# lmjakt/kmer_hasheR

Measured on AMD Instinct MI355X. Metric: Mbp/s indexed (make.kmer.hash k=31) at 1/2/4/8 GPUs; seq.kmer.pos query Mbp/s, higher is better.
Workload: dtype u64; 1 GPU; configs[1]: synthetic 10 Mbp iid ACGT (splitmix64 seed 1+rank), k=31, make.kmer.hash index build; self seq.kmer.pos query timed alongside; seq_len=10000000, k=31, distinct_kmers=9999970, positions=9999970, parallelism=single

## Files before the change

### kmer_hasher_amd/csrc/kmhg_engine.cpp

```cpp
#include <atomic>
#include <hip/hip_runtime.h>
#include <sys/mman.h>

#include <algorithm>
#include <climits>
#include <cmath>
#include <cstdio>
#include <cstdlib>
#include <cstring>
#include <exception>
#include <functional>
#include <map>
#include <memory>
#include <mutex>
#include <numeric>
#include <string>
#include <thread>
#include <vector>

#include "kmhg_common.h"
#include "kmhg_blocks.h"
#include "kmhg_chains.h"
#include "kmhg_kernels.h"
#include "kmhg_plan.h"
#include "kmhg_hostwork.h"
#include "kmhg_pool.h"
#include "kmhg_reads.h"
#include "kmhg_querycall.h"
#include "kmhg_segrec.h"
#include "kmhg_parts_read.h"
#include "kmhg_fastx.h"
#include "kmhg_khash.h"
#include "kmhg_sh.h"

namespace kmhg {
inline const char* test_build_knob(const char* name) {
#ifdef KMHG_TEST_BUILD
  return std::getenv(name);
#else
  (void)name;
  return nullptr;
#endif
}
}
#include "../../include/kmhgpu.h"

using namespace kmhg;

static thread_local std::string g_err;

namespace {

struct Error {
  int code;
  std::string msg;
};

[[noreturn]] void fail(int code, const std::string& msg) { throw Error{code, msg}; }

void hip_check(hipError_t e, const char* what) {
  if (e != hipSuccess) {
    if (e == hipErrorOutOfMemory) fail(KMHG_ENOMEM, std::string(what) + ": out of device memory");
    fail(KMHG_EDEVICE, std::string(what) + ": " + hipGetErrorString(e));
  }
}
#define HIPC(x) hip_check((x), #x)

template <class F>
int guarded(F&& f) {
  try {
    f();
    return KMHG_OK;
  } catch (const Error& e) {
    g_err = e.msg;
    return e.code;
  } catch (const std::bad_alloc&) {
    g_err = "host allocation failed";
    return KMHG_ENOMEM;
  }
}

struct HipDev {
  static PoolKnobs knobs() {
    PoolKnobs kn;
    if (const char* e = test_build_knob("KMHG_POOL_DEPTH"))
      kn.depth = (size_t)std::max(1, std::min(8, std::atoi(e)));
    if (const char* e = test_build_knob("KMHG_POOL_BESTFIT")) kn.best_fit = e[0] != '0';
    kn.trace = test_build_knob("KMHG_POOL_TRACE") != nullptr;
    return kn;
  }
  int current() { int dev = 0; HIPC(hipGetDevice(&dev)); return dev; }
  void use(int dev) { (void)hipSetDevice(dev); }
  PoolAlloc alloc(size_t sz, void** p, std::string* text) {
    const hipError_t e = hipMalloc(p, sz);
    if (e == hipSuccess) return PoolAlloc::ok;
    if (e == hipErrorOutOfMemory) { (void)hipGetLastError(); return PoolAlloc::oom; }
    *text = hipGetErrorString(e);
    return PoolAlloc::error;
  }
  void free(void* p) { (void)hipFree(p); }
  void* event() {
    hipEvent_t ev = nullptr;
    if (hipEventCreateWithFlags(&ev, hipEventDisableTiming | hipEventDisableSystemFence) ==
        hipSuccess)
      return ev;
    (void)hipGetLastError();
    return hipEventCreateWithFlags(&ev, hipEventDisableTiming) == hipSuccess ? ev : nullptr;
  }
  bool record(void* ev, void* s) {
    return hipEventRecord(static_cast<hipEvent_t>(ev), static_cast<hipStream_t>(s)) == hipSuccess;
  }
  bool done(void* ev) { return hipEventQuery(static_cast<hipEvent_t>(ev)) == hipSuccess; }
  void wait_event(void* ev) { (void)hipEventSynchronize(static_cast<hipEvent_t>(ev)); }
  void wait_stream(void* s) { (void)hipStreamSynchronize(static_cast<hipStream_t>(s)); }
  [[noreturn]] void alloc_failed(PoolAlloc st, const std::string& text) {
    if (st == PoolAlloc::oom) fail(KMHG_ENOMEM, "hipMalloc: out of device memory");
    fail(KMHG_EDEVICE, "hipMalloc: " + text);
  }
};
using DevicePool = BlockPool<HipDev>;
using ReleaseGroup = ReleaseGroupT<HipDev>;

template <class T>
struct DBuf {
  T* p = nullptr;
  size_t n = 0;
  hipStream_t s = nullptr;
  bool ordered = false;
  DBuf() = default;
  explicit DBuf(size_t count) { reset(count); }
  DBuf(size_t count, hipStream_t stream) { reset(count); bind(stream); }
  ~DBuf() { free(); }
  DBuf(const DBuf&) = delete;
  DBuf& operator=(const DBuf&) = delete;
  void bind(hipStream_t stream) { s = stream; ordered = true; }
  void reset(size_t count) {
    free();
    n = count;
    p = static_cast<T*>(DevicePool::get().alloc(std::max<size_t>(count, 1) * sizeof(T)));
  }
  void free() {
    if (p) DevicePool::get().release(p, s, ordered);
    p = nullptr; n = 0;
  }
  size_t bytes() const { return n * sizeof(T); }
  void swap_with(DBuf& o) {
    std::swap(p, o.p);
    std::swap(n, o.n);
    std::swap(s, o.s);
    std::swap(ordered, o.ordered);
  }
};

struct PinnedRec {
  BuildMeta* meta = nullptr;
  hipEvent_t ev = nullptr;
};
class PinnedPool {
 public:
  static PinnedPool& get() {
    static PinnedPool p;
    return p;
  }
  PinnedRec take() {
    std::lock_guard<std::mutex> g(mu_);
    for (size_t i = 0; i < pending_.size();) {
      if (hipEventQuery(pending_[i].ev) == hipSuccess) {
        free_.push_back(pending_[i]);
        pending_[i] = pending_.back();
        pending_.pop_back();
      } else {
        ++i;
      }
    }
    if (free_.empty()) {
      constexpr int kSlots = 64;
      BuildMeta* blk = nullptr;
      HIPC(hipHostMalloc(reinterpret_cast<void**>(&blk), sizeof(BuildMeta) * kSlots,
                         hipHostMallocCoherent));
      for (int i = 0; i < kSlots; ++i) {
        PinnedRec r;
        r.meta = blk + i;
        HIPC(hipEventCreateWithFlags(&r.ev, hipEventDisableTiming));
        free_.push_back(r);
      }
    }
    PinnedRec r = free_.back();
    free_.pop_back();
    std::memset(r.meta, 0, sizeof(*r.meta));
    return r;
  }
  void give(PinnedRec r, bool in_flight) {
    if (!r.meta) return;
    std::lock_guard<std::mutex> g(mu_);
    (in_flight ? pending_ : free_).push_back(r);
  }

 private:
  std::mutex mu_;
  std::vector<PinnedRec> free_, pending_;
};
struct GiveBack {
  PinnedRec& r;
  hipStream_t s;
  ~GiveBack() {
    if (std::uncaught_exceptions() > 0) (void)hipStreamSynchronize(s);
    PinnedPool::get().give(r, false);
  }
};

struct Timing {
  static Timing& get() {
    static Timing t;
    return t;
  }
  bool on = false;
  std::string only;
  struct Rec { std::string name; hipEvent_t a, b; };
  std::vector<Rec> recs;
  std::map<std::string, std::pair<int64_t, double>> acc;
  std::mutex mu;

  Timing() {
    const char* e = std::getenv("KMHG_TIMING");
    on = e && e[0] == '1';
  }
  std::vector<hipEvent_t> pool;
  hipEvent_t take() {
    if (!pool.empty()) { hipEvent_t e = pool.back(); pool.pop_back(); return e; }
    hipEvent_t e;
    if (hipEventCreateWithFlags(&e, hipEventDisableSystemFence) != hipSuccess) {
      (void)hipGetLastError();
      HIPC(hipEventCreate(&e));
    }
    return e;
  }
  template <class F>
  void run(const char* name, hipStream_t s, F&& launch) {
    if (!on || (!only.empty() && only != name)) { launch(); HIPC(hipGetLastError()); return; }
    hipEvent_t a, b;
    {
      std::lock_guard<std::mutex> g(mu);
      a = take();
      b = take();
    }
    HIPC(hipEventRecord(a, s));
    launch();
    HIPC(hipGetLastError());
    HIPC(hipEventRecord(b, s));
    std::lock_guard<std::mutex> g(mu);
    recs.push_back({name, a, b});
  }
  void collect() {
    std::lock_guard<std::mutex> g(mu);
    for (auto& r : recs) {
      (void)hipEventSynchronize(r.b);
      float ms = 0.f;
      (void)hipEventElapsedTime(&ms, r.a, r.b);
      auto& x = acc[r.name];
      x.first += 1;
      x.second += ms;
      pool.push_back(r.a);
      pool.push_back(r.b);
    }
    recs.clear();
  }
};
#define LAUNCH(name, stream, ...) Timing::get().run(name, stream, [&] { __VA_ARGS__; })

hipStream_t lib_stream() {
  static std::mutex mu;
  static std::map<int, hipStream_t> streams;
  int dev = 0;
  HIPC(hipGetDevice(&dev));
  std::lock_guard<std::mutex> g(mu);
  auto it = streams.find(dev);
  if (it != streams.end()) return it->second;
  hipStream_t s;
  HIPC(hipStreamCreateWithFlags(&s, hipStreamNonBlocking));
  streams[dev] = s;
  return s;
}

static bool fresh_threads() {
  const char* pe = test_build_knob("KMHG_HOST_POOL");
  return pe && pe[0] == '0';
}

constexpr size_t D2H_CHUNK = 16u << 20;
constexpr size_t D2H_STAGE_MIN = 4u << 20;
static int d2h_threads() {
  static const int n = [] {
    const char* e = std::getenv("KMHG_D2H_THREADS");
    return e ? std::max(1, std::min(16, std::atoi(e))) : 8;
  }();
  return n;
}

static void host_copy_par(char* dst, const char* src, size_t n) {
  for_stripes(n, d2h_threads(), 4096, fresh_threads(),
              [=](uint64_t a, uint64_t b) { std::memcpy(dst + a, src + a, b - a); });
}

struct PinStage {
  std::mutex mu;
  char* pin[2] = {nullptr, nullptr};
};
static PinStage& pin_stage() {
  static std::mutex map_mu;
  static std::map<int, PinStage> stages;
  int dev = 0;
  HIPC(hipGetDevice(&dev));
  std::lock_guard<std::mutex> g(map_mu);
  return stages[dev];
}

static void hint_huge_pages(void* dst, size_t bytes) {
  static const bool on = [] {
    const char* e = test_build_knob("KMHG_D2H_HUGE");
    return !(e && e[0] == '0');
  }();
  const Span h = on ? huge_span(dst, bytes) : Span{0, 0};
  if (h.len) (void)madvise(reinterpret_cast<void*>(h.begin), h.len, MADV_HUGEPAGE);
}

void d2h_host(void* dst, const void* src, size_t bytes, hipStream_t s) {
  if (!bytes) return;
  static const bool staged = [] {
    const char* e = test_build_knob("KMHG_D2H");
    return !(e && std::string(e) == "direct");
  }();
  hint_huge_pages(dst, bytes);
  if (!staged || bytes < D2H_STAGE_MIN) {
    HIPC(hipMemcpyAsync(dst, src, bytes, hipMemcpyDeviceToHost, s));
    HIPC(hipStreamSynchronize(s));
    return;
  }
  PinStage& st = pin_stage();
  std::lock_guard<std::mutex> g(st.mu);
  char** pin = st.pin;
  if (!pin[0])
    for (int i = 0; i < 2; ++i)
      HIPC(hipHostMalloc(reinterpret_cast<void**>(&pin[i]), D2H_CHUNK, hipHostMallocPortable));
  struct Ev2 {
    hipEvent_t e[2] = {nullptr, nullptr};
    hipStream_t s;
    ~Ev2() {
      if (std::uncaught_exceptions() > 0) (void)hipStreamSynchronize(s);
      for (auto x : e)
        if (x) (void)hipEventDestroy(x);
    }
  } evs{{nullptr, nullptr}, s};
  hipEvent_t* ev = evs.e;
// ... 217 lines not shown
    }
  });
  const size_t n = effective_len(seq, L);
  copy.join();
  if (err.code != KMHG_OK) fail(err.code, err.msg);
  return n;
}

void check_build_args(size_t L, int k) {
  if (k < 1 || k > 32) fail(KMHG_EINVAL, "k must be a positive integer less than 1+MAX_K");
  if ((int64_t)L <= k) fail(KMHG_EINVAL, "the length of the sequence must be at least k");
  if (L >= (size_t)INT32_MAX) fail(KMHG_EOVERFLOW, "sequence longer than 2^31-1 (int positions)");
}

QueryCall checked(const QueryCall& c) {
  if (c.code != KMHG_OK) fail(c.code, c.text);
  return c;
}

void check_query_args(size_t L, int k) { checked(query_call(L, k)); }

template <class F>
Error for_parts(const std::vector<int>& key, F&& fn) {
  const int n = (int)key.size();
  std::vector<Error> errs(n, Error{KMHG_OK, ""});
  std::vector<int> uniq;
  for (int d : key)
    if (std::find(uniq.begin(), uniq.end(), d) == uniq.end()) uniq.push_back(d);
  auto run_key = [&](int d) {
    for (int i = 0; i < n; ++i) {
      if (key[i] != d) continue;
      try {
        fn(i);
      } catch (const Error& e) {
        errs[i] = e;
      } catch (const std::bad_alloc&) {
        errs[i] = Error{KMHG_ENOMEM, "host allocation failed"};
      }
    }
  };
  std::vector<std::thread> th;
  for (size_t u = 1; u < uniq.size(); ++u) th.emplace_back(run_key, uniq[u]);
  if (!uniq.empty()) run_key(uniq[0]);
  for (auto& t : th) t.join();
  for (const Error& e : errs)
    if (e.code != KMHG_OK) return e;
  return Error{KMHG_OK, ""};
}

kmhg_index* build_device_v1(const uint8_t* d_seq, int64_t L, int k, hipStream_t s) {
  ReleaseGroup rg(s);
  auto idx = std::make_unique<kmhg_index>();
  idx->stream = s;
  idx->build_kind = KMHG_BUILD_GLOBAL;
  HIPC(hipGetDevice(&idx->device));
  idx->k = k;
  idx->L = L;
  const int64_t Nw = L - k + 1;
  const bool aligned = (reinterpret_cast<uintptr_t>(d_seq) & 15) == 0;
  idx->geom = Geom{1u, (uint32_t)table_capacity(Nw)};
  const uint64_t nslots = idx->slots();
  idx->table.reset(nslots);
  DBuf<uint32_t> win_slot(Nw, s);
  LAUNCH("k_table_init", s, launch_table_init(idx->table.p, nslots, s));
  LAUNCH("k_build_insert", s,
         launch_build_insert(d_seq, L, k, idx->table.p, idx->geom, win_slot.p, Nw, aligned, s));
  const uint32_t nt = tiles_for(nslots);
  const size_t scratch_bytes = (size_t)nt * 8 + 64 + sizeof(BuildMeta);
  DBuf<uint8_t> scratch(scratch_bytes, s);
  HIPC(hipMemsetAsync(scratch.p, 0, scratch_bytes, s));
  uint64_t* status = reinterpret_cast<uint64_t*>(scratch.p);
  uint32_t* ticket = reinterpret_cast<uint32_t*>(scratch.p + (size_t)nt * 8);
  BuildMeta* meta = reinterpret_cast<BuildMeta*>(scratch.p + (size_t)nt * 8 + 64);
  DBuf<uint64_t> ukeys(Nw, s);
  DBuf<uint32_t> counts(Nw, s), offsets(Nw + 1, s);
  DBuf<uint32_t> small_ids(Nw / 2 + 1, s), large_ids(Nw / LARGE_MIN + 1, s);
  LAUNCH("k_build_compact", s,
         launch_build_compact(idx->table.p, nslots, status, ticket, ukeys.p, counts.p,
                              offsets.p, small_ids.p, large_ids.p, meta, s));
  idx->positions.reset(Nw);
  LAUNCH("k_build_scatter", s, launch_build_scatter(win_slot.p, Nw, idx->table.p,
                                                    idx->positions.p, s));
  LAUNCH("k_sort_small", s, launch_sort_small(small_ids.p, meta, counts.p, offsets.p,
                                              idx->positions.p, s));
  LAUNCH("k_sort_large", s,
         launch_sort_large(large_ids.p, meta, counts.p, offsets.p, idx->positions.p,
                           reinterpret_cast<int32_t*>(win_slot.p), s));
  LAUNCH("k_inline_singles", s, launch_inline_singles(idx->table.p, nslots, idx->positions.p, s));
  BuildMeta hm;
  HIPC(hipMemcpyAsync(&hm, meta, sizeof(hm), hipMemcpyDeviceToHost, s));
  HIPC(hipStreamSynchronize(s));
  idx->U = hm.n_kmers;
  idx->N = hm.n_positions;
  idx->P = hm.n_pairs;
  idx->max_n = hm.max_count;
  return idx.release();
}

BuildKnobs read_build_knobs() {
  BuildKnobs kn;
  for (const char* name : BUILD_KNOB_NAMES)
    if (const char* v = test_build_knob(name)) set_build_knob(kn, name, v);
  return kn;
}

uint32_t bucket_round_of_current_device() {
  static std::atomic<uint32_t> cache[64];
  int dev = 0;
  if (hipGetDevice(&dev) != hipSuccess || dev < 0) return 0;
  if (dev < 64) {
    if (uint32_t v = cache[dev].load(std::memory_order_relaxed)) return v;
  }
  int cus = 0;
  if (hipDeviceGetAttribute(&cus, hipDeviceAttributeMultiprocessorCount, dev) != hipSuccess)
    cus = 0;
  const uint32_t v = (uint32_t)std::max(cus, 0) * (uint32_t)KMHG_BUCKET_WGS;
  if (dev < 64) cache[dev].store(v, std::memory_order_relaxed);
  return v;
}

#ifdef KMHG_TEST_BUILD
static std::mutex g_place_mu;
static uint32_t* g_place_ctr = nullptr;
static int g_place_dev = -1;
uint32_t* bucket_place_counters() {
  std::lock_guard<std::mutex> lk(g_place_mu);
  int dev = 0;
  HIPC(hipGetDevice(&dev));
  if (!g_place_ctr) {
    HIPC(hipMalloc(&g_place_ctr, 3 * sizeof(uint32_t)));
    HIPC(hipMemset(g_place_ctr, 0, 3 * sizeof(uint32_t)));
    g_place_dev = dev;
  }
  return dev == g_place_dev ? g_place_ctr : nullptr;
}
#else
uint32_t* bucket_place_counters() { return nullptr; }
#endif

#ifdef KMHG_TEST_BUILD
static std::atomic<uint64_t> g_bid_pack_ctr[2];
void count_bid_pack(bool packed) { g_bid_pack_ctr[packed ? 0 : 1].fetch_add(1, std::memory_order_relaxed); }
#else
void count_bid_pack(bool) {}
#endif

struct StreamPtrs {
  const uint8_t* d_seq = nullptr;
  const uint64_t* d_keys = nullptr;
};

kmhg_index* build_device_v2(const BuildRequest& rq, const StreamPtrs& in, hipStream_t s) {
  ReleaseGroup rg(s);
  const BuildKnobs kn = read_build_knobs();
  const BuildPlan P = plan_build(rq, kn, bucket_round_of_current_device());
  if (P.err != KMHG_OK) fail(P.err, P.msg);
  auto idx = std::make_unique<kmhg_index>();
  idx->stream = s;
  HIPC(hipGetDevice(&idx->device));
  idx->build_kind = ballot_ranks() ? KMHG_BUILD_PARTITIONED_BALLOT : KMHG_BUILD_PARTITIONED;
  idx->k = rq.k;
  idx->L = rq.L;
  idx->is_part = P.is_part;
  idx->geom = P.geom;
  if (P.empty_part) {
    idx->table.reset(1);
    idx->positions.reset(1);
    return idx.release();
  }
  const int k = rq.k;
  const int64_t L = rq.L, Nw = P.Nw;
  const bool from_keys = P.from_keys, co_auto = P.co_auto, bid = P.bid, partc = P.partc;
  const uint32_t passes = P.passes, R = P.R, ntiles = P.ntiles, nb = P.geom.nb;
  const uint64_t nhist = P.nhist;
  const Geom g = P.geom;
  auto mk_digit = [&](uint32_t dv, uint32_t r) { return make_digit(dv, r, P.digit32 ? g.nb : 0u); };
  const uint64_t* d_keys = in.d_keys;
  const uint8_t* d_seq = in.d_seq;
  DBuf<uint8_t> aligned_copy;
  if (!from_keys && (reinterpret_cast<uintptr_t>(d_seq) & 15) != 0) {
    aligned_copy.reset((size_t)L);
    aligned_copy.bind(s);
    HIPC(hipMemcpyAsync(aligned_copy.p, d_seq, (size_t)L, hipMemcpyDeviceToDevice, s));
    d_seq = aligned_copy.p;
  }
  if (bid) count_bid_pack(P.bid_pack);
  auto kwords = [&](int sd) { return ((uint64_t)(Nw + PTILE) * P.key_bytes[sd] + 7) / 8; };
  DBuf<uint64_t> kA(kwords(0), s), kB(kwords(1), s);
  DBuf<uint32_t> pA(P.pos_array[0] ? Nw + PTILE : 1, s), pB(P.pos_array[1] ? Nw + PTILE : 1, s);
  auto kptr = [&](int p) -> void* {
    return p < 0 && from_keys ? const_cast<uint64_t*>(d_keys) : P.side(p) ? kB.p : kA.p;
  };
  auto pptr = [&](int p) { return P.side(p) ? pB.p : pA.p; };
  const uint32_t pad = (uint32_t)Nw;
  DBuf<uint32_t> hist(nhist, s);
  DBuf<uint32_t> start((uint64_t)nb + 1, s);
  DBuf<uint32_t> segb(P.pack8 ? (uint64_t)R * (P.nseg8 + 1) : 1, s);
  DBuf<uint16_t> dsb(P.ds_on ? ((uint64_t)Nw + PTILE + 8) / (P.ds8 ? 2 : 1) + 8 : 1, s);
  uint8_t* ds8p = P.ds8 ? reinterpret_cast<uint8_t*>(dsb.p) : nullptr;
  uint16_t* ds16p = P.ds8 ? nullptr : dsb.p;
  const Pack8 pk8{P.pack8 ? P.sh8 : 0, segb.p, P.nseg8, mk_digit(1, R)};
  const size_t off_meta = 64, off_status = 128;
  const uint32_t n_status = P.scan_tiles + 1;
  const size_t scratch_bytes = off_status + (size_t)n_status * 8;
  DBuf<uint8_t> scratch(scratch_bytes, s);
  uint8_t* sc = scratch.p;
  uint32_t* n_valid = reinterpret_cast<uint32_t*>(sc);
  BuildMeta* meta = reinterpret_cast<BuildMeta*>(sc + off_meta);
  uint64_t* status = reinterpret_cast<uint64_t*>(sc + off_status);
  idx->rec = PinnedPool::get().take();
  if (!co_auto) idx->table.reset(idx->slots());
  idx->positions.reset(P.no_pos ? 1 : Nw);
  idx->bstats.reset(nb);
  DBuf<uint32_t> hll_rows(co_auto ? (size_t)ntiles * (HLL_REGS / 4) : 1, s);
  DBuf<uint32_t> hll_regs(co_auto ? HLL_PART_WORDS : 1, s);
  PinnedRec hrec;
  if (co_auto) hrec = PinnedPool::get().take();

  DBuf<uint32_t> lo_save(passes >= 2 ? R : 1, s);
  uint64_t r_top = 1;
  for (uint32_t i = 1; i < passes; ++i) r_top *= R;
  DBuf<uint32_t> lvA(passes >= 3 ? r_top + 1 : 1, s), lvB(passes >= 4 ? r_top + 1 : 1, s);
  uint32_t div = 1;
  DiagBlock db{nullptr, nullptr, nullptr};
  DBuf<uint32_t> tcnt(partc ? ntiles : 1, s);
  if (from_keys) {
    HIPC(hipMemsetD32Async(reinterpret_cast<hipDeviceptr_t>(n_valid), (int)Nw, 1, s));
    HIPC(hipMemsetAsync(meta, 0, sizeof(BuildMeta), s));
  } else {
    if (rq.codes) {
      idx->dcodes.reset(diag_block_words(Nw));
      db = idx->diag_block_of();
    }
    LAUNCH("k_v2_hist0", s,
           launch_v2_hist0(d_seq, L, k, Nw, g, mk_digit(1, R), hist.p, ntiles, status,
                           n_status, meta, s, db.code, db.nbit,
                           bid ? static_cast<uint32_t*>(kptr(-1)) : nullptr,
                           partc ? kB.p : nullptr, partc ? pB.p : nullptr,
                           partc ? tcnt.p : nullptr));
    if (partc) {
      LAUNCH("k_scan_u32", s, launch_scan_u32(tcnt.p, ntiles, status, n_valid, s));
    } else {
      LAUNCH("k_scan_u32", s, launch_scan_u32(hist.p, nhist, status, n_valid, s));
      const DigitOut ds0{ds16p, mk_digit(R, R), ds8p};
      LAUNCH("k_v2_scatter_seq", s,
             launch_v2_scatter(bid ? ScatterIn::first_pass(kptr(-1), Nw)
                                   : ScatterIn::sequence(d_seq, L, k, Nw),
                               P.F(-1), P.F(0), kptr(0), pptr(0), pad, n_valid, g, mk_digit(1, R),
                               hist.p, ntiles, s, nullptr, P.pack8 ? &pk8 : nullptr,
                               P.ds_out(0) ? &ds0 : nullptr));
      if (P.pack8)
        LAUNCH("k_seg_bounds", s,
               launch_seg_bounds(hist.p, ntiles, R, P.nseg8, (uint32_t)(P.seg8 / PTILE), n_valid,
                                 segb.p, s));
      div = R;
    }
  }
  uint32_t* hp = hist.p;
  uint32_t C = ntiles, nst = n_status;
  uint64_t nh = nhist;
  DBuf<uint32_t> hist1;
  if (rq.n_parts >= 2 && (passes > 1 || partc)) {
    uint32_t nv = 0;
    HIPC(hipMemcpyAsync(&nv, n_valid, 4, hipMemcpyDeviceToHost, s));
    HIPC(hipStreamSynchronize(s));
    C = std::max<uint32_t>(1u, (uint32_t)(((uint64_t)nv + PTILE - 1) / PTILE));
    nh = (uint64_t)R * C;
    nst = tiles_for(nh) + 1;
    hist1.reset(nh);
    hist1.bind(s);
    hp = hist1.p;
    if (!partc)
      HIPC(hipMemcpy2DAsync(lo_save.p, 4, hist.p, (size_t)ntiles * 4, 4, R,
                            hipMemcpyDeviceToDevice, s));
  }
  if (partc)
    LAUNCH("k_part_dense", s, launch_part_dense(kB.p, pB.p, tcnt.p, ntiles, n_valid, kptr(-1),
                                                pptr(-1), P.F(-1), s));
  uint32_t* save1 = hp == hist.p || partc ? lo_save.p : nullptr;
  auto level_of = [&](uint32_t p, uint32_t spread) {
    uint64_t dv = 1;
    for (uint32_t i = 0; i < p; ++i) dv *= R;
    const bool last = p + 1 == passes;
    const uint32_t* lin = p == 1 ? lo_save.p : ((p - 1) % 2 ? lvA.p : lvB.p);
    uint32_t* lout = last ? start.p : (p % 2 ? lvA.p : lvB.p);
    return BoundsFuse{lin, lout, mk_digit((uint32_t)dv, R), (uint32_t)dv, spread,
                      last ? g.nb : (uint32_t)(dv * R)};
  };
  auto launch_level = [&](uint32_t p, const BoundsFuse& f) {
    LAUNCH("k_v2_bounds", s,
           launch_v2_bounds_lo(P.F((int)p - 1), kptr((int)p - 1), n_valid, g, f.Dlast, f.div, hp, C,
                               f.lo_start, f.spread, f.start, f.nlim, s, pk8.sh));
  };
  for (uint32_t p = P.first_pass; p < passes; ++p) {
    const Digit Dp = mk_digit(div, R);
    const bool keys0 = from_keys && p == 0;
    const bool last = p + 1 == passes;
    const bool hll = co_auto && p == 0;
    const int pi = (int)p - 1;
    if (keys0)
      LAUNCH("k_v2_hist", s,
             launch_v2_hist_keys0(d_keys, n_valid, g, Dp, hp, C, status, nst, s,
                                  hll ? hll_rows.p : nullptr, hll ? hll_regs.p : nullptr,
                                  rq.skip_empty));
    else
      LAUNCH("k_v2_hist", s,
             launch_v2_hist(!P.ds_out(pi) ? P.F(pi)
                            : P.ds8       ? StreamFmt::Digits8
                                          : StreamFmt::Digits16,
                            P.ds_out(pi) ? dsb.p : kptr(pi), n_valid, g, Dp, hp, C, status, nst, s,
                            p == 1 ? save1 : nullptr, pk8.sh));
    LAUNCH("k_scan_u32", s, launch_scan_u32(hp, nh, status, n_valid, s));
    if (hll) {
      LAUNCH("k_v2_hll", s, launch_v2_hll(hll_rows.p, ntiles, hll_regs.p,
                                          &hrec.meta->distinct_est, n_valid,
                                          &hrec.meta->n_positions, s));
      HIPC(hipEventRecord(hrec.ev, s));
    }
    const BoundsFuse lv = level_of(p, 1u);
    const DigitOut dsn{ds16p, mk_digit(div * R, R), ds8p};
    LAUNCH("k_v2_scatter", s,
           launch_v2_scatter(keys0 ? ScatterIn::first_pass(d_keys, Nw, rq.skip_empty)
                                   : ScatterIn::stream(kptr(pi), pptr(pi)),
                             P.F(pi), P.F((int)p), kptr((int)p), pptr((int)p), pad, n_valid, g, Dp,
                             hp, C, s, P.fused(p) ? &lv : nullptr, P.pack8 ? &pk8 : nullptr,
                             P.ds_out((int)p) ? &dsn : nullptr));
    if (p >= 1 && !P.fused(p) && !last) launch_level(p, lv);
    div *= R;
  }
  const int last_p = (int)passes - 1;
  Geom gb = g;
  if (co_auto) {
    HIPC(hipEventSynchronize(hrec.ev));
    idx->co_est = hrec.meta->distinct_est;
    const uint64_t n_keys_valid = hrec.meta->n_positions;
    PinnedPool::get().give(hrec, false);
    idx->co_spread = co_spread_for(idx->co_est, n_keys_valid, kn.co_spread);
    gb = Geom{nb / (uint32_t)idx->co_spread, V2_CAPW};
    idx->geom = gb;
    idx->table.reset(idx->slots());
  }
  if (passes == 1) {
    LAUNCH("k_v2_bounds", s,
           launch_v2_bounds_lo(StreamFmt::Keys, nullptr, n_valid, g, mk_digit(1, R), 1u,
                               partc ? hp : hist.p, partc ? C : ntiles, nullptr, g.nb / gb.nb,
                               start.p, g.nb, s));
  } else if (!P.fused(passes - 1)) {
    launch_level(passes - 1, level_of(passes - 1, g.nb / gb.nb));
  }
#ifdef KMHG_STAMPS
  static uint64_t* stamps = nullptr;
  if (!stamps) HIPC(hipMallocManaged(&stamps, sizeof(uint64_t) * 8 * (1u << 22)));
  HIPC(hipMemsetAsync(stamps, 0, sizeof(uint64_t) * 8 * nb, s));
  kmhg::set_stamp_buffer(stamps);
#endif
  if (kn.test_disorder && !P.no_pos)
    launch_v2_test_disorder(P.F(last_p), kptr(last_p), pptr(last_p), start.p, n_valid,
                            kn.test_disorder, s);
  uint8_t* tg = nullptr;
  uint32_t* rep = nullptr;
  if (P.want_tags) {
    try {
      idx->ptag.reset(idx->slots() + 32);
      idx->ptag.bind(s);
      tg = idx->ptag.p;
      rep = db.uniq;
      HIPC(hipMemsetAsync(rep, 0, diag_uniq_words(Nw) * 4, s));
      HIPC(hipMemsetAsync(tg + idx->slots() - 1, 0, 33, s));
    } catch (const Error& e) {
      if (e.code != KMHG_ENOMEM) throw;
      (void)hipGetLastError();
      tg = nullptr;
      rep = nullptr;
    }
  }
  LAUNCH("k_v2_bucket_wg", s,
         launch_v2_bucket_wg(P.F(last_p), kptr(last_p), pptr(last_p), start.p, gb, idx->table.p,
                             idx->positions.p, idx->bstats.p, meta, s, n_valid, (uint32_t)Nw,
                             db.code, k, tg, rep, kn.bucket_place, bucket_place_counters()));
  idx->tags_built = tg != nullptr;
  LAUNCH("k_v2_stats", s, launch_v2_stats(idx->bstats.p, gb.nb, n_valid, meta, idx->rec.meta, s));
  idx->bstats_nb = gb.nb;
  HIPC(hipEventRecord(idx->rec.ev, s));
  rg.adopt(idx->rec.ev);
#ifdef KMHG_STAMPS
  if (const char* f = std::getenv("KMHG_STAMP_FILE")) {
    HIPC(hipStreamSynchronize(s));
    if (FILE* fp = fopen(f, "wb")) { fwrite(stamps, 8, 8 * (size_t)nb, fp); fclose(fp); }
  }
#endif
  idx->pending = true;
  idx->src = in.d_seq;
  return idx.release();
}

bool tags_on() {
  const char* e = test_build_knob("KMHG_QUERY_TAGS");
  return !(e && e[0] == '0');
}

static std::atomic<int> g_lane_state[64];
static std::mutex g_lane_mu;
static void lane_order_run(int blocks, uint64_t* bad, uint64_t* checked) {
  struct Probe {
    hipStream_t st = nullptr;
    unsigned long long* res = nullptr;
  };
  static Probe probes[64];
  int dev = 0;
  HIPC(hipGetDevice(&dev));
  Probe& pr = probes[(unsigned)dev % 64];
  if (!pr.st) HIPC(hipStreamCreateWithFlags(&pr.st, hipStreamNonBlocking));
  if (!pr.res) HIPC(hipMalloc(&pr.res, 2 * sizeof(unsigned long long)));
  unsigned long long h[2] = {0, 0};
  hipError_t e = hipMemsetAsync(pr.res, 0, sizeof(h), pr.st);
  if (e == hipSuccess) {
    launch_lane_order_check(pr.res, pr.st, blocks);
    e = hipMemcpyAsync(h, pr.res, sizeof(h), hipMemcpyDeviceToHost, pr.st);
  }
  if (e == hipSuccess) e = hipStreamSynchronize(pr.st);
  hip_check(e, "LDS lane-order check");
  *bad = h[0];
  *checked = h[1];
}
bool lane_ballot() {
  if (const char* e = test_build_knob("KMHG_TEST_BALLOT"))
    if (e[0] == '1') return true;
  int dev = 0;
  HIPC(hipGetDevice(&dev));
  std::atomic<int>& st = g_lane_state[(unsigned)dev % 64];
  int v = st.load(std::memory_order_acquire);
  if (v == 0) {
    std::lock_guard<std::mutex> lk(g_lane_mu);
    v = st.load(std::memory_order_relaxed);
    if (v == 0) {
      uint64_t bad = 0, chk = 0;
      lane_order_run(256, &bad, &chk);
      v = (bad == 0 && chk > 0) ? 1 : 2;
      st.store(v, std::memory_order_release);
    }
  }
  return v == 2;
}

int build_version() {
  const char* e = test_build_knob("KMHG_BUILD");
  return (e && std::string(e) == "v1") ? 1 : 2;
}

kmhg_index* build_device(const uint8_t* d_seq, int64_t L, int k, hipStream_t s, bool codes = true) {
  if (const char* e = test_build_knob("KMHG_DIAG_CODES"))
    if (e[0] == '0') codes = false;
  if (build_version() == 2)
    return build_device_v2(BuildRequest::sequence(L, k, codes), StreamPtrs{d_seq, nullptr}, s);
  return build_device_v1(d_seq, L, k, s);
}

void finish_build(kmhg_index* idx) {
  if (!idx->pending) return;
  HIPC(hipEventSynchronize(idx->rec.ev));
  const BuildMeta hm = *idx->rec.meta;
  PinnedPool::get().give(idx->rec, false);
  idx->rec = PinnedRec{};
  idx->pending = false;
  const uint8_t* src = idx->src;
  idx->src = nullptr;
  if (hm.overflow) {
    if (idx->is_part) fail(KMHG_EOVERFLOW, "a bucket of a part build overflowed its LDS table");
    std::unique_ptr<kmhg_index> v1(build_device_v1(src, idx->L, idx->k, idx->stream));
    idx->build_kind = KMHG_BUILD_GLOBAL;
    idx->tags_built = false;
    idx->bstats_nb = 0;
    idx->fallback = 1;
    idx->geom = v1->geom;
    idx->table.swap_with(v1->table);
    idx->positions.swap_with(v1->positions);
    idx->U = v1->U; idx->N = v1->N; idx->P = v1->P; idx->max_n = v1->max_n;
    v1->table.bind(idx->stream);
    v1->positions.bind(idx->stream);
    return;
  }
  idx->U = hm.n_kmers;
  idx->N = hm.n_positions;
  idx->P = hm.n_pairs;
  idx->max_n = hm.max_count;
}

bool ensure_diag(kmhg_index* idx, hipStream_t s) {
  if (idx->ps_ready.load(std::memory_order_acquire)) return true;
  std::lock_guard<std::mutex> lk(idx->ps_mu);
  if (idx->ps_ready.load(std::memory_order_relaxed) || idx->ps_failed) return !idx->ps_failed;
  if (!idx->tags_built) {
    try {
      idx->ptag.reset(idx->slots() + 32);
    } catch (const Error& e) {
      if (e.code != KMHG_ENOMEM) throw;
      idx->ps_failed = true;
      (void)hipGetLastError();
      return false;
    }
    idx->ptag.bind(s);
  }
  idx->dcodes.bind(s);
  const DiagBlock db = idx->diag_block_of();
  if (idx->tags_built)
    LAUNCH("k_diag_valid", s, launch_diag_valid(db.nbit, idx->L, idx->k, db.uniq, true, s));
  else
    LAUNCH("k_diag_prep", s,
           launch_diag_prep(db.nbit, idx->L, idx->k, db.uniq, idx->table.p, idx->slots(),
                            idx->positions.p, idx->ptag.p, s));
  HIPC(hipStreamSynchronize(s));
  idx->ps_ready.store(true, std::memory_order_release);
  return true;
}

kmhg_query* query_device(kmhg_index* idx, const uint8_t* d_seq, const QueryCall& c,
                         hipStream_t s) {
// ... 2965 lines not shown
```

### kmer_hasher_amd/csrc/kmhg_pool.h

```cpp
#pragma once
#include <stdint.h>

#include <algorithm>
#include <cstdio>
#include <map>
#include <mutex>
#include <string>
#include <utility>
#include <vector>

namespace kmhg {

inline size_t pool_size_class(size_t b) {
  if (b <= (1u << 20)) {
    size_t r = 256;
    while (r < b) r <<= 1;
    return r;
  }
  const size_t g = 2u << 20;
  return (b + g - 1) / g * g;
}

struct PoolKnobs {
  size_t depth = 1;
  bool best_fit = true;
  bool trace = false;
};

enum class PoolAlloc { ok, oom, error };

template <class Dev>
struct ReleaseGroupT;

template <class Dev>
class BlockPool {
 public:
  using Key = std::pair<int, size_t>;
  struct Block { void* p; Key key; void* ev; bool owns_ev; };
  struct Snapshot {
    std::vector<Block> live, free, pending;
    size_t idle_events, cached;
  };

  explicit BlockPool(PoolKnobs kn = {}, Dev dev = {}) : kn_(kn), dev_(dev) {}
  BlockPool(const BlockPool&) = delete;
  BlockPool& operator=(const BlockPool&) = delete;
  static BlockPool& get() {
    static BlockPool p(Dev::knobs());
    return p;
  }

  void* alloc(size_t bytes) {
    if (bytes == 0) bytes = 256;
    const Key key{dev_.current(), pool_size_class(bytes)};
    const size_t sz = key.second;
    {
      std::unique_lock<std::mutex> g(mu_);
      poll_pending();
      auto fl = free_.find(key);
      if (fl != free_.end() && !fl->second.empty()) return take(fl);
      auto n = count_.find(key);
      if (n != count_.end() && n->second >= kn_.depth) {
        for (size_t i = 0; i < pending_.size(); ++i) {
          if (pending_[i].key != key) continue;
          const Block pd = pending_[i];
          pending_.erase(pending_.begin() + (long)i);
          g.unlock();
          dev_.wait_event(pd.ev);
          g.lock();
          if (pd.owns_ev) events_.push_back(pd.ev);
          live_[pd.p] = pd.key;
          return pd.p;
        }
      }
      if (kn_.best_fit && sz >= BEST_FIT_MIN) {
        for (auto it = free_.lower_bound(key);
             it != free_.end() && it->first.first == key.first && it->first.second <= sz + sz / 2;
             ++it)
          if (!it->second.empty()) return take(it);
      }
    }
    if (kn_.trace)
      std::fprintf(stderr, "kmhg pool: hipMalloc %zu B on device %d\n", sz, key.first);
    void* p = nullptr;
    std::string text;
    PoolAlloc st = dev_.alloc(sz, &p, &text);
    if (st == PoolAlloc::oom) {
      trim();
      st = dev_.alloc(sz, &p, &text);
    }
    if (st != PoolAlloc::ok) dev_.alloc_failed(st, text);
    std::lock_guard<std::mutex> g(mu_);
    live_[p] = key;
    ++count_[key];
    return p;
  }

  void release(void* p, void* stream = nullptr, bool ordered = false) {
    if (!p) return;
    ReleaseGroupT<Dev>* rg = ReleaseGroupT<Dev>::open;
    if (ordered && rg && &rg->pool == this && rg->s == stream) {
      rg->ps.push_back(p);
      return;
    }
    if (ordered) release_behind(&p, 1, stream);
    else release_now(&p, 1);
  }
  void release_behind(void* const* ps, size_t n, void* stream, void* adopted = nullptr) {
    if (n == 0) return;
    if (adopted) {
      std::lock_guard<std::mutex> g(mu_);
      for (size_t i = 0; i < n; ++i) retire(ps[i], adopted);
      return;
    }
    void* ev = recorded_event(stream);
    std::lock_guard<std::mutex> g(mu_);
    const size_t before = pending_.size();
    for (size_t i = 0; i < n; ++i) retire(ps[i], ev);
    if (!ev) return;
    if (pending_.size() > before) pending_.back().owns_ev = true;
    else events_.push_back(ev);
  }
  void release_now(void* const* ps, size_t n) {
    std::lock_guard<std::mutex> g(mu_);
    for (size_t i = 0; i < n; ++i) retire(ps[i], nullptr);
  }
  void trim() {
    std::lock_guard<std::mutex> g(mu_);
    for (const Block& pd : pending_) {
      dev_.wait_event(pd.ev);
      settle(pd);
    }
    pending_.clear();
    const int cur = dev_.current();
    for (auto& kv : free_) {
      dev_.use(kv.first.first);
      for (void* p : kv.second) dev_.free(p);
      auto n = count_.find(kv.first);
      if (n != count_.end()) n->second -= std::min(n->second, kv.second.size());
      cached_ -= kv.first.second * kv.second.size();
    }
    free_.clear();
    dev_.use(cur);
  }
  int64_t cached() {
    std::lock_guard<std::mutex> g(mu_);
    return (int64_t)cached_;
  }
  Snapshot snapshot() {
    std::lock_guard<std::mutex> g(mu_);
    Snapshot s{{}, {}, pending_, events_.size(), cached_};
    for (auto& kv : live_) s.live.push_back({kv.first, kv.second, nullptr, false});
    for (auto& kv : free_)
      for (void* p : kv.second) s.free.push_back({p, kv.first, nullptr, false});
    return s;
  }

 private:
  using FreeLists = std::map<Key, std::vector<void*>>;
  void* take(typename FreeLists::iterator fl) {
    void* p = fl->second.back();
    fl->second.pop_back();
    cached_ -= fl->first.second;
    live_[p] = fl->first;
    return p;
  }
  void retire(void* p, void* ev) {
    auto it = live_.find(p);
    if (it == live_.end()) return;
    const Block b{p, it->second, ev, false};
    live_.erase(it);
    if (ev) pending_.push_back(b);
    else settle(b);
  }
  void settle(const Block& b) {
    if (b.owns_ev) events_.push_back(b.ev);
    free_[b.key].push_back(b.p);
    cached_ += b.key.second;
  }
  void poll_pending() {
    for (size_t i = 0; i < pending_.size();) {
      if (dev_.done(pending_[i].ev)) {
        settle(pending_[i]);
        pending_[i] = pending_.back();
        pending_.pop_back();
      } else {
        ++i;
      }
    }
  }
  void* recorded_event(void* stream) {
    void* ev = nullptr;
    {
      std::lock_guard<std::mutex> g(mu_);
      if (!events_.empty()) { ev = events_.back(); events_.pop_back(); }
    }
    if (!ev) ev = dev_.event();
    if (!ev || !dev_.record(ev, stream)) {
      dev_.wait_stream(stream);
      if (ev) { std::lock_guard<std::mutex> g(mu_); events_.push_back(ev); }
      ev = nullptr;
    }
    return ev;
  }

  static constexpr size_t BEST_FIT_MIN = (size_t)256 << 20;
  const PoolKnobs kn_;
  Dev dev_;
  std::mutex mu_;
  FreeLists free_;
  std::map<Key, size_t> count_;
  std::map<void*, Key> live_;
  std::vector<Block> pending_;
  std::vector<void*> events_;
  size_t cached_ = 0;
};

template <class Dev>
struct ReleaseGroupT {
  static inline thread_local ReleaseGroupT* open = nullptr;
  BlockPool<Dev>& pool;
  void* s;
  std::vector<void*> ps;
  ReleaseGroupT* prev;
  bool synced = false;
  void* adopted = nullptr;
  ReleaseGroupT(BlockPool<Dev>& pl, void* stream) : pool(pl), s(stream), prev(open) { open = this; }
  explicit ReleaseGroupT(void* stream) : ReleaseGroupT(BlockPool<Dev>::get(), stream) {}
  ~ReleaseGroupT() {
    open = prev;
    if (synced) pool.release_now(ps.data(), ps.size());
    else pool.release_behind(ps.data(), ps.size(), s, adopted);
  }
  void adopt(void* ev) { adopted = ev; }
  ReleaseGroupT(const ReleaseGroupT&) = delete;
  ReleaseGroupT& operator=(const ReleaseGroupT&) = delete;
};

}
```

Measured before the change: 60220 Mbp/s.

## Reuse device blocks pending on the same stream and bound pinned record lookahead

The device block pool now records the stream each pending block was released on. An allocation on that same stream can reclaim such a block immediately, because stream ordering makes reuse safe without waiting on the event. poll_pending caches event query results so a shared event is checked only once. Pinned metadata records move into a RecordPool that caps the number in flight and waits on the oldest one beyond that cap. All build buffers are allocated with the stream hint, which is meant to cut hipMalloc calls and event polling in the host-side allocation path, at the risk of blocking when the lookahead cap is reached.

Result: faster. 64260 Mbp/s (median of 6 runs) (+6.7%).

```diff
diff --git a/kmer_hasher_amd/csrc/kmhg_engine.cpp b/kmer_hasher_amd/csrc/kmhg_engine.cpp
--- a/kmer_hasher_amd/csrc/kmhg_engine.cpp
+++ b/kmer_hasher_amd/csrc/kmhg_engine.cpp
@@ -85,6 +85,9 @@
     PoolKnobs kn;
     if (const char* e = test_build_knob("KMHG_POOL_DEPTH"))
       kn.depth = (size_t)std::max(1, std::min(8, std::atoi(e)));
+    if (const char* e = test_build_knob("KMHG_POOL_AHEAD"))
+      kn.ahead = (size_t)std::max(1, std::min(8, std::atoi(e)));
+    if (const char* e = test_build_knob("KMHG_POOL_STREAM")) kn.same_stream = e[0] != '0';
     if (const char* e = test_build_knob("KMHG_POOL_BESTFIT")) kn.best_fit = e[0] != '0';
     kn.trace = test_build_knob("KMHG_POOL_TRACE") != nullptr;
     return kn;
@@ -120,6 +123,10 @@
 };
 using DevicePool = BlockPool<HipDev>;
 using ReleaseGroup = ReleaseGroupT<HipDev>;
+
+struct FirstUseOn {
+  hipStream_t s;
+};
 
 template <class T>
 struct DBuf {
@@ -130,6 +137,7 @@
   DBuf() = default;
   explicit DBuf(size_t count) { reset(count); }
   DBuf(size_t count, hipStream_t stream) { reset(count); bind(stream); }
+  DBuf(size_t count, FirstUseOn on) { reset(count, on); }
   ~DBuf() { free(); }
   DBuf(const DBuf&) = delete;
   DBuf& operator=(const DBuf&) = delete;
@@ -138,6 +146,12 @@
     free();
     n = count;
     p = static_cast<T*>(DevicePool::get().alloc(std::max<size_t>(count, 1) * sizeof(T)));
+  }
+  void reset(size_t count, FirstUseOn on) {
+    free();
+    n = count;
+    p = static_cast<T*>(DevicePool::get().alloc(std::max<size_t>(count, 1) * sizeof(T), on.s));
+    bind(on.s);
   }
   void free() {
     if (p) DevicePool::get().release(p, s, ordered);
@@ -163,17 +177,7 @@
     return p;
   }
   PinnedRec take() {
-    std::lock_guard<std::mutex> g(mu_);
-    for (size_t i = 0; i < pending_.size();) {
-      if (hipEventQuery(pending_[i].ev) == hipSuccess) {
-        free_.push_back(pending_[i]);
-        pending_[i] = pending_.back();
-        pending_.pop_back();
-      } else {
-        ++i;
-      }
-    }
-    if (free_.empty()) {
+    PinnedRec r = recs_.take([](std::vector<PinnedRec>& out) {
       constexpr int kSlots = 64;
       BuildMeta* blk = nullptr;
       HIPC(hipHostMalloc(reinterpret_cast<void**>(&blk), sizeof(BuildMeta) * kSlots,
@@ -182,23 +186,19 @@
         PinnedRec r;
         r.meta = blk + i;
         HIPC(hipEventCreateWithFlags(&r.ev, hipEventDisableTiming));
-        free_.push_back(r);
+        out.push_back(r);
       }
-    }
-    PinnedRec r = free_.back();
-    free_.pop_back();
+    });
     std::memset(r.meta, 0, sizeof(*r.meta));
     return r;
   }
   void give(PinnedRec r, bool in_flight) {
     if (!r.meta) return;
-    std::lock_guard<std::mutex> g(mu_);
-    (in_flight ? pending_ : free_).push_back(r);
+    recs_.give(r, in_flight);
   }
 
  private:
-  std::mutex mu_;
-  std::vector<PinnedRec> free_, pending_;
+  RecordPool<HipDev, PinnedRec> recs_{HipDev::knobs().ahead};
 };
 struct GiveBack {
   PinnedRec& r;
@@ -722,6 +722,7 @@
 
 kmhg_index* build_device_v2(const BuildRequest& rq, const StreamPtrs& in, hipStream_t s) {
   ReleaseGroup rg(s);
+  const FirstUseOn on{s};
   const BuildKnobs kn = read_build_knobs();
   const BuildPlan P = plan_build(rq, kn, bucket_round_of_current_device());
   if (P.err != KMHG_OK) fail(P.err, P.msg);
@@ -749,57 +750,56 @@
   const uint8_t* d_seq = in.d_seq;
   DBuf<uint8_t> aligned_copy;
   if (!from_keys && (reinterpret_cast<uintptr_t>(d_seq) & 15) != 0) {
-    aligned_copy.reset((size_t)L);
-    aligned_copy.bind(s);
+    aligned_copy.reset((size_t)L, on);
     HIPC(hipMemcpyAsync(aligned_copy.p, d_seq, (size_t)L, hipMemcpyDeviceToDevice, s));
     d_seq = aligned_copy.p;
   }
   if (bid) count_bid_pack(P.bid_pack);
   auto kwords = [&](int sd) { return ((uint64_t)(Nw + PTILE) * P.key_bytes[sd] + 7) / 8; };
-  DBuf<uint64_t> kA(kwords(0), s), kB(kwords(1), s);
-  DBuf<uint32_t> pA(P.pos_array[0] ? Nw + PTILE : 1, s), pB(P.pos_array[1] ? Nw + PTILE : 1, s);
+  DBuf<uint64_t> kA(kwords(0), on), kB(kwords(1), on);
+  DBuf<uint32_t> pA(P.pos_array[0] ? Nw + PTILE : 1, on), pB(P.pos_array[1] ? Nw + PTILE : 1, on);
   auto kptr = [&](int p) -> void* {
     return p < 0 && from_keys ? const_cast<uint64_t*>(d_keys) : P.side(p) ? kB.p : kA.p;
   };
   auto pptr = [&](int p) { return P.side(p) ? pB.p : pA.p; };
   const uint32_t pad = (uint32_t)Nw;
-  DBuf<uint32_t> hist(nhist, s);
-  DBuf<uint32_t> start((uint64_t)nb + 1, s);
-  DBuf<uint32_t> segb(P.pack8 ? (uint64_t)R * (P.nseg8 + 1) : 1, s);
-  DBuf<uint16_t> dsb(P.ds_on ? ((uint64_t)Nw + PTILE + 8) / (P.ds8 ? 2 : 1) + 8 : 1, s);
+  DBuf<uint32_t> hist(nhist, on);
+  DBuf<uint32_t> start((uint64_t)nb + 1, on);
+  DBuf<uint32_t> segb(P.pack8 ? (uint64_t)R * (P.nseg8 + 1) : 1, on);
+  DBuf<uint16_t> dsb(P.ds_on ? ((uint64_t)Nw + PTILE + 8) / (P.ds8 ? 2 : 1) + 8 : 1, on);
   uint8_t* ds8p = P.ds8 ? reinterpret_cast<uint8_t*>(dsb.p) : nullptr;
   uint16_t* ds16p = P.ds8 ? nullptr : dsb.p;
   const Pack8 pk8{P.pack8 ? P.sh8 : 0, segb.p, P.nseg8, mk_digit(1, R)};
   const size_t off_meta = 64, off_status = 128;
   const uint32_t n_status = P.scan_tiles + 1;
   const size_t scratch_bytes = off_status + (size_t)n_status * 8;
-  DBuf<uint8_t> scratch(scratch_bytes, s);
+  DBuf<uint8_t> scratch(scratch_bytes, on);
   uint8_t* sc = scratch.p;
   uint32_t* n_valid = reinterpret_cast<uint32_t*>(sc);
   BuildMeta* meta = reinterpret_cast<BuildMeta*>(sc + off_meta);
   uint64_t* status = reinterpret_cast<uint64_t*>(sc + off_status);
   idx->rec = PinnedPool::get().take();
-  if (!co_auto) idx->table.reset(idx->slots());
-  idx->positions.reset(P.no_pos ? 1 : Nw);
-  idx->bstats.reset(nb);
-  DBuf<uint32_t> hll_rows(co_auto ? (size_t)ntiles * (HLL_REGS / 4) : 1, s);
-  DBuf<uint32_t> hll_regs(co_auto ? HLL_PART_WORDS : 1, s);
+  if (!co_auto) idx->table.reset(idx->slots(), on);
+  idx->positions.reset(P.no_pos ? 1 : Nw, on);
+  idx->bstats.reset(nb, on);
+  DBuf<uint32_t> hll_rows(co_auto ? (size_t)ntiles * (HLL_REGS / 4) : 1, on);
+  DBuf<uint32_t> hll_regs(co_auto ? HLL_PART_WORDS : 1, on);
   PinnedRec hrec;
   if (co_auto) hrec = PinnedPool::get().take();
 
-  DBuf<uint32_t> lo_save(passes >= 2 ? R : 1, s);
+  DBuf<uint32_t> lo_save(passes >= 2 ? R : 1, on);
   uint64_t r_top = 1;
   for (uint32_t i = 1; i < passes; ++i) r_top *= R;
-  DBuf<uint32_t> lvA(passes >= 3 ? r_top + 1 : 1, s), lvB(passes >= 4 ? r_top + 1 : 1, s);
+  DBuf<uint32_t> lvA(passes >= 3 ? r_top + 1 : 1, on), lvB(passes >= 4 ? r_top + 1 : 1, on);
   uint32_t div = 1;
   DiagBlock db{nullptr, nullptr, nullptr};
-  DBuf<uint32_t> tcnt(partc ? ntiles : 1, s);
+  DBuf<uint32_t> tcnt(partc ? ntiles : 1, on);
   if (from_keys) {
     HIPC(hipMemsetD32Async(reinterpret_cast<hipDeviceptr_t>(n_valid), (int)Nw, 1, s));
     HIPC(hipMemsetAsync(meta, 0, sizeof(BuildMeta), s));
   } else {
     if (rq.codes) {
-      idx->dcodes.reset(diag_block_words(Nw));
+      idx->dcodes.reset(diag_block_words(Nw), on);
       db = idx->diag_block_of();
     }
     LAUNCH("k_v2_hist0", s,
@@ -837,8 +837,7 @@
     C = std::max<uint32_t>(1u, (uint32_t)(((uint64_t)nv + PTILE - 1) / PTILE));
     nh = (uint64_t)R * C;
     nst = tiles_for(nh) + 1;
-    hist1.reset(nh);
-    hist1.bind(s);
+    hist1.reset(nh, on);
     hp = hist1.p;
     if (!partc)
       HIPC(hipMemcpy2DAsync(lo_save.p, 4, hist.p, (size_t)ntiles * 4, 4, R,
@@ -908,7 +907,7 @@
     idx->co_spread = co_spread_for(idx->co_est, n_keys_valid, kn.co_spread);
     gb = Geom{nb / (uint32_t)idx->co_spread, V2_CAPW};
     idx->geom = gb;
-    idx->table.reset(idx->slots());
+    idx->table.reset(idx->slots(), on);
   }
   if (passes == 1) {
     LAUNCH("k_v2_bounds", s,
@@ -931,8 +930,7 @@
   uint32_t* rep = nullptr;
   if (P.want_tags) {
     try {
-      idx->ptag.reset(idx->slots() + 32);
-      idx->ptag.bind(s);
+      idx->ptag.reset(idx->slots() + 32, on);
       tg = idx->ptag.p;
       rep = db.uniq;
       HIPC(hipMemsetAsync(rep, 0, diag_uniq_words(Nw) * 4, s));
diff --git a/kmer_hasher_amd/csrc/kmhg_pool.h b/kmer_hasher_amd/csrc/kmhg_pool.h
--- a/kmer_hasher_amd/csrc/kmhg_pool.h
+++ b/kmer_hasher_amd/csrc/kmhg_pool.h
@@ -23,6 +23,8 @@
 
 struct PoolKnobs {
   size_t depth = 1;
+  size_t ahead = 2;
+  bool same_stream = true;
   bool best_fit = true;
   bool trace = false;
 };
@@ -36,7 +38,7 @@
 class BlockPool {
  public:
   using Key = std::pair<int, size_t>;
-  struct Block { void* p; Key key; void* ev; bool owns_ev; };
+  struct Block { void* p; Key key; void* ev; bool owns_ev; void* stream = nullptr; };
   struct Snapshot {
     std::vector<Block> live, free, pending;
     size_t idle_events, cached;
@@ -50,12 +52,21 @@
     return p;
   }
 
-  void* alloc(size_t bytes) {
+  void* alloc(size_t bytes) { return alloc_for(bytes, false, nullptr); }
+  void* alloc(size_t bytes, void* stream) { return alloc_for(bytes, kn_.same_stream, stream); }
+
+ private:
+  void* alloc_for(size_t bytes, bool on_stream, void* stream) {
     if (bytes == 0) bytes = 256;
     const Key key{dev_.current(), pool_size_class(bytes)};
     const size_t sz = key.second;
     {
       std::unique_lock<std::mutex> g(mu_);
+      if (on_stream) {
+        auto fl = free_.find(key);
+        if (fl != free_.end() && !fl->second.empty()) return take(fl);
+        if (void* p = take_pending_of(key, stream)) return p;
+      }
       poll_pending();
       auto fl = free_.find(key);
       if (fl != free_.end() && !fl->second.empty()) return take(fl);
@@ -96,6 +107,7 @@
     return p;
   }
 
+ public:
   void release(void* p, void* stream = nullptr, bool ordered = false) {
     if (!p) return;
     ReleaseGroupT<Dev>* rg = ReleaseGroupT<Dev>::open;
@@ -110,13 +122,13 @@
     if (n == 0) return;
     if (adopted) {
       std::lock_guard<std::mutex> g(mu_);
-      for (size_t i = 0; i < n; ++i) retire(ps[i], adopted);
+      for (size_t i = 0; i < n; ++i) retire(ps[i], adopted, stream);
       return;
     }
     void* ev = recorded_event(stream);
     std::lock_guard<std::mutex> g(mu_);
     const size_t before = pending_.size();
-    for (size_t i = 0; i < n; ++i) retire(ps[i], ev);
+    for (size_t i = 0; i < n; ++i) retire(ps[i], ev, stream);
     if (!ev) return;
     if (pending_.size() > before) pending_.back().owns_ev = true;
     else events_.push_back(ev);
@@ -150,9 +162,9 @@
   Snapshot snapshot() {
     std::lock_guard<std::mutex> g(mu_);
     Snapshot s{{}, {}, pending_, events_.size(), cached_};
-    for (auto& kv : live_) s.live.push_back({kv.first, kv.second, nullptr, false});
+    for (auto& kv : live_) s.live.push_back({kv.first, kv.second, nullptr, false, nullptr});
     for (auto& kv : free_)
-      for (void* p : kv.second) s.free.push_back({p, kv.first, nullptr, false});
+      for (void* p : kv.second) s.free.push_back({p, kv.first, nullptr, false, nullptr});
     return s;
   }
 
@@ -165,10 +177,10 @@
     live_[p] = fl->first;
     return p;
   }
-  void retire(void* p, void* ev) {
+  void retire(void* p, void* ev, void* stream = nullptr) {
     auto it = live_.find(p);
     if (it == live_.end()) return;
-    const Block b{p, it->second, ev, false};
+    const Block b{p, it->second, ev, false, stream};
     live_.erase(it);
     if (ev) pending_.push_back(b);
     else settle(b);
@@ -178,9 +190,33 @@
     free_[b.key].push_back(b.p);
     cached_ += b.key.second;
   }
+  void* take_pending_of(const Key& key, void* stream) {
+    for (size_t i = 0; i < pending_.size(); ++i) {
+      if (pending_[i].key != key || pending_[i].stream != stream) continue;
+      const Block pd = pending_[i];
+      pending_.erase(pending_.begin() + (long)i);
+      if (pd.owns_ev) {
+        size_t heir = pending_.size();
+        for (size_t j = 0; j < pending_.size() && heir == pending_.size(); ++j)
+          if (pending_[j].ev == pd.ev) heir = j;
+        if (heir < pending_.size()) pending_[heir].owns_ev = true;
+        else events_.push_back(pd.ev);
+      }
+      live_[pd.p] = pd.key;
+      return pd.p;
+    }
+    return nullptr;
+  }
   void poll_pending() {
+    std::vector<std::pair<void*, bool>> seen;
+    const auto done = [&](void* ev) {
+      for (const auto& e : seen)
+        if (e.first == ev) return e.second;
+      seen.emplace_back(ev, dev_.done(ev));
+      return seen.back().second;
+    };
     for (size_t i = 0; i < pending_.size();) {
-      if (dev_.done(pending_[i].ev)) {
+      if (done(pending_[i].ev)) {
         settle(pending_[i]);
         pending_[i] = pending_.back();
         pending_.pop_back();
@@ -237,4 +273,51 @@
   ReleaseGroupT& operator=(const ReleaseGroupT&) = delete;
 };
 
+template <class Dev, class Rec>
+class RecordPool {
+ public:
+  explicit RecordPool(size_t ahead = PoolKnobs{}.ahead, Dev dev = {})
+      : ahead_(std::max<size_t>(ahead, 1)), dev_(dev) {}
+  RecordPool(const RecordPool&) = delete;
+  RecordPool& operator=(const RecordPool&) = delete;
+  template <class Grow>
+  Rec take(Grow&& grow) {
+    std::unique_lock<std::mutex> g(mu_);
+    for (size_t i = 0; i < pending_.size();) {
+      if (dev_.done(pending_[i].ev)) {
+        free_.push_back(pending_[i]);
+        pending_.erase(pending_.begin() + (long)i);
+      } else {
+        ++i;
+      }
+    }
+    while (pending_.size() >= ahead_) {
+      const Rec r = pending_.front();
+      pending_.erase(pending_.begin());
+      g.unlock();
+      dev_.wait_event(r.ev);
+      g.lock();
+      free_.push_back(r);
+    }
+    if (free_.empty()) grow(free_);
+    const Rec r = free_.back();
+    free_.pop_back();
+    return r;
+  }
+  void give(const Rec& r, bool in_flight) {
+    std::lock_guard<std::mutex> g(mu_);
+    (in_flight ? pending_ : free_).push_back(r);
+  }
+  std::pair<size_t, size_t> sizes() {
+    std::lock_guard<std::mutex> g(mu_);
+    return {free_.size(), pending_.size()};
+  }
+
+ private:
+  const size_t ahead_;
+  Dev dev_;
+  std::mutex mu_;
+  std::vector<Rec> free_, pending_;
+};
+
 }
```
